# Lapis-Hong/wide_deep

Hardware: NVIDIA H100
Metric: CTR examples/sec (train step) (higher is better)
Workload: dtype bf16x3 (fp32 operands split into bf16 hi+lo, 3 tensor-core products, fp32 accumulate; 2^-16)

## Files before the change

wide_deep_b200/csrc/gemm.cuh:

```cuda
#pragma once
#include <cuda.h>
#include <cuda_bf16.h>

#include "common.cuh"

namespace wd {

__device__ __forceinline__ float act_fwd(int kind, float z) {
    switch (kind) {
        case WD_ACT_RELU: return fmaxf(z, 0.f);
        case WD_ACT_RELU6: return fminf(fmaxf(z, 0.f), 6.f);
        case WD_ACT_SIGMOID: return 1.f / (1.f + expf(-z));
        case WD_ACT_TANH: return tanhf(z);
        case WD_ACT_LEAKY_RELU: return z > 0.f ? z : 0.2f * z;
        case WD_ACT_ELU: return z > 0.f ? z : expm1f(z);
        case WD_ACT_SELU: return 1.0507009873554805f * (z > 0.f ? z : 1.6732632423543772f * expm1f(z));
        case WD_ACT_SOFTPLUS: return fmaxf(z, 0.f) + log1pf(expf(-fabsf(z)));
        case WD_ACT_SOFTSIGN: return z / (1.f + fabsf(z));
    }
    return z;
}
__device__ __forceinline__ float act_bwd(int kind, float a) {
    switch (kind) {
        case WD_ACT_RELU: return a > 0.f ? 1.f : 0.f;
        case WD_ACT_RELU6: return (a > 0.f && a < 6.f) ? 1.f : 0.f;
        case WD_ACT_SIGMOID: return a * (1.f - a);
        case WD_ACT_TANH: return 1.f - a * a;
        case WD_ACT_LEAKY_RELU: return a > 0.f ? 1.f : 0.2f;
        case WD_ACT_ELU: return a > 0.f ? 1.f : a + 1.f;
        case WD_ACT_SELU: return a > 0.f ? 1.0507009873554805f : a + 1.0507009873554805f * 1.6732632423543772f;
        case WD_ACT_SOFTPLUS: return 1.f - expf(-a);
        case WD_ACT_SOFTSIGN: { float t = 1.f - fabsf(a); return t * t; }
    }
    return 1.f;
}

struct GemmA {
    int n;
    const float* ptr[kMaxSegs];
    int ld[kMaxSegs];
    int k[kMaxSegs];
    const __nv_bfloat16* hi[kMaxSegs];
    const __nv_bfloat16* lo[kMaxSegs];
};
struct GemmB {
    const float* ptr; int ld;
    const float *tf32_hi, *tf32_lo;
    const __nv_bfloat16 *hi, *lo;
};
enum { EPI_FWD = 0, EPI_STORE = 1, EPI_WGRAD = 2 };
struct Epi {
    float* C; int ldc;
    int accumulate;
    float* A_out; float* H_out; int ldh;
    float* HT; int ldt;
    const float *bias, *gamma, *beta;
    int n_logical, act, bn;
    int m_valid;
    int64_t split_stride;
    __nv_bfloat16 *Hs_hi, *Hs_lo;
    uint64_t reserved[5];
};

int tc_gemm(WdModel* m, int mode, const GemmA& A, const GemmB& B, int M, int N, const Epi& ep, int splits, int ksplit_len);
int tc_gemm_bf16(WdModel* m, int mode, const GemmA& A, const GemmB& B, int M, int N, const Epi& ep, int splits, int ksplit_len);
int make_tensor_map(CUtensorMap* map, CUtensorMapDataType dtype, const void* ptr, int rows, int cols, int ld, int box_rows);

struct DropArgs { float rate; unsigned long long seed; const unsigned int* step; int layer_id; unsigned int row0; };
__device__ __forceinline__ unsigned long long splitmix64_dev(unsigned long long x) {
    x += 0x9E3779B97F4A7C15ULL;
    x = (x ^ (x >> 30)) * 0xBF58476D1CE4E5B9ULL;
    x = (x ^ (x >> 27)) * 0x94D049BB133111EBULL;
    return x ^ (x >> 31);
}
__device__ __forceinline__ unsigned long long drop_key(const DropArgs& d) {
    return splitmix64_dev(d.seed ^ ((unsigned long long)(*d.step) * 0x9E3779B97F4A7C15ULL) ^ ((unsigned long long)d.layer_id << 48));
}
__device__ __forceinline__ float drop_mult(unsigned long long key, unsigned int m, unsigned int n, float rate, float inv_keep) {
    const unsigned long long r = splitmix64_dev(key ^ ((unsigned long long)m * 65536ULL + n));
    const float u = (float)(unsigned int)(r >> 40) * (1.f / 16777216.f);
    return u >= rate ? inv_keep : 0.f;
}

__device__ __forceinline__ float bn_out(float a, const float* __restrict__ gamma, const float* __restrict__ beta, int n, int bn) {
    return bn ? fmaf(a, gamma[n] * 0.99950037468777f, beta[n]) : a;
}

__device__ __forceinline__ void split_bf16(float x, __nv_bfloat16& hi, __nv_bfloat16& lo) {
    hi = __float2bfloat16_rn(x);
    lo = __float2bfloat16_rn(x - __bfloat162float(hi));
}
__device__ __forceinline__ void split_pair(float x0, float x1, uint32_t& hi, uint32_t& lo) {
    const __nv_bfloat162 hp = __floats2bfloat162_rn(x0, x1);
    hi = *reinterpret_cast<const uint32_t*>(&hp);
    const __nv_bfloat162 lp = __floats2bfloat162_rn(x0 - __uint_as_float(hi << 16), x1 - __uint_as_float(hi & 0xFFFF0000u));
    lo = *reinterpret_cast<const uint32_t*>(&lp);
}
__device__ __forceinline__ void store_split4(__nv_bfloat16* hi, __nv_bfloat16* lo, float x0, float x1, float x2, float x3) {
    uint2 ph, pl;
    split_pair(x0, x1, ph.x, pl.x);
    split_pair(x2, x3, ph.y, pl.y);
    *reinterpret_cast<uint2*>(hi) = ph;
    *reinterpret_cast<uint2*>(lo) = pl;
}

}
```

wide_deep_b200/csrc/gemm_bf16.cu:

```cuda
#include <cuda.h>
#include <stdlib.h>

#include <algorithm>
#include <type_traits>

#include "common.cuh"
#include "gemm.cuh"
#include "wgmma_ptx.cuh"

namespace wd {

namespace {

constexpr int QBM = 128;
constexpr int QBN = 128;
constexpr int QNST = 3;
constexpr int QBK = 64;
constexpr int Q_THREADS = 384;

struct QMaps {
    CUtensorMap a_hi[kMaxSegs], a_lo[kMaxSegs];
    CUtensorMap b_hi, b_lo;
};
struct QSegs { int n; int k[kMaxSegs]; int koff[kMaxSegs]; };

__device__ unsigned long long g_probe[32 * 8];
__device__ __forceinline__ unsigned long long gtime() { unsigned long long t; asm volatile("mov.u64 %0, %globaltimer;" : "=l"(t)); return t; }
#define PROBE(i) do { if (probe >= 0 && blockIdx.x == 0 && (threadIdx.x & 127) == 0) g_probe[probe * 8 + (i)] = gtime(); } while (0)

template <int MODE>
__global__ void __launch_bounds__(Q_THREADS, 1) tc_gemm_bf16_kernel(const __grid_constant__ QMaps maps, const QSegs segs, int M, int N, int ktot,
                                                                   int ksplit_len, int nsplit, Epi ep, int probe) {
    extern __shared__ uint8_t smem_raw[];
    uint8_t* base = reinterpret_cast<uint8_t*>((reinterpret_cast<uintptr_t>(smem_raw) + 1023) & ~uintptr_t(1023));
    constexpr bool A_MN = MODE == EPI_WGRAD;
    constexpr bool B_MN = MODE == EPI_FWD || MODE == EPI_WGRAD;
    constexpr int A_BYTES = QBM * 128, B_BYTES = QBN * 128;
    constexpr int STAGE_BYTES = 2 * (A_BYTES + B_BYTES);
    auto a_hi = [&](int s) { return base + s * STAGE_BYTES; };
    auto a_lo = [&](int s) { return base + s * STAGE_BYTES + A_BYTES; };
    auto b_hi = [&](int s) { return base + s * STAGE_BYTES + 2 * A_BYTES; };
    auto b_lo = [&](int s) { return base + s * STAGE_BYTES + 2 * A_BYTES + B_BYTES; };
    uint64_t* bars = reinterpret_cast<uint64_t*>(base + QNST * STAGE_BYTES);
    uint64_t* full = bars; uint64_t* empty = bars + QNST;
    float* epi_vec = reinterpret_cast<float*>(base + QNST * STAGE_BYTES + 64);

    const int warp = threadIdx.x >> 5, lane = threadIdx.x & 31, wg = threadIdx.x >> 7;
    const int tiles_n = (N + QBN - 1) / QBN, tiles_m = (M + QBM - 1) / QBM;
    const int ntiles = tiles_n * tiles_m * nsplit;
    int nkb_all = 0;
    for (int s = 0; s < segs.n; ++s) nkb_all += (segs.k[s] + QBK - 1) / QBK;
    auto tile_range = [&](int tile, int& m0, int& n0, int& z, int& kbeg, int& nkb) {
        z = tile / (tiles_n * tiles_m);
        int r = tile % (tiles_n * tiles_m);
        m0 = (r / tiles_n) * QBM;
        n0 = (r % tiles_n) * QBN;
        kbeg = 0;
        nkb = nkb_all;
        if (MODE == EPI_WGRAD) {
            kbeg = z * ksplit_len;
            int kend = min(ktot, kbeg + ksplit_len);
            nkb = kend > kbeg ? (kend - kbeg + QBK - 1) / QBK : 0;
        }
    };

    if (threadIdx.x == 0) {
        for (int s = 0; s < QNST; ++s) { mbar_init(&full[s], 1); mbar_init(&empty[s], 8); }
        asm volatile("fence.mbarrier_init.release.cluster;" ::: "memory");
    }
    __syncthreads();

    if (wg == 0) {
        reg_dealloc<40>();
        PROBE(0);
        if (warp == 0 && lane == 0) {
            int g = 0;
            for (int tile = blockIdx.x; tile < ntiles; tile += gridDim.x) {
                int m0, n0, z, kbeg, nkb;
                tile_range(tile, m0, n0, z, kbeg, nkb);
                int seg = 0, kin = 0;
                for (int kb = 0; kb < nkb; ++kb, ++g) {
                    const int s = g % QNST, it = g / QNST;
                    if (it > 0) mbar_wait(&empty[s], (it - 1) & 1);
                    int ka, kbcoord;
                    if (MODE == EPI_WGRAD) { ka = kbeg + kb * QBK; kbcoord = ka; }
                    else {
                        if (kin >= segs.k[seg]) { ++seg; kin = 0; }
                        ka = kin; kbcoord = segs.koff[seg] + kin;
                        kin += QBK;
                    }
                    mbar_expect_tx(&full[s], 2 * (A_BYTES + B_BYTES));
                    if (!A_MN) {
                        tma_load_2d(a_hi(s), &maps.a_hi[seg], &full[s], ka, m0);
                        tma_load_2d(a_lo(s), &maps.a_lo[seg], &full[s], ka, m0);
                    } else {
#pragma unroll
                        for (int i = 0; i < QBM / 64; ++i) {
                            tma_load_2d(a_hi(s) + i * 8192, &maps.a_hi[seg], &full[s], m0 + 64 * i, ka);
                            tma_load_2d(a_lo(s) + i * 8192, &maps.a_lo[seg], &full[s], m0 + 64 * i, ka);
                        }
                    }
                    if (!B_MN) {
                        tma_load_2d(b_hi(s), &maps.b_hi, &full[s], kbcoord, n0);
                        tma_load_2d(b_lo(s), &maps.b_lo, &full[s], kbcoord, n0);
                    } else {
#pragma unroll
                        for (int i = 0; i < QBN / 64; ++i) {
                            tma_load_2d(b_hi(s) + i * 8192, &maps.b_hi, &full[s], n0 + 64 * i, kbcoord);
                            tma_load_2d(b_lo(s) + i * 8192, &maps.b_lo, &full[s], n0 + 64 * i, kbcoord);
                        }
                    }
                }
            }
        }
    } else {
        reg_alloc<232>();
        const int cw = wg - 1, cwarp = warp - 4;
        constexpr uint32_t a_step = A_MN ? 2048u : 32u, b_step = B_MN ? 2048u : 32u;
        constexpr int TA = A_MN ? 1 : 0, TB = B_MN ? 1 : 0;
        float d[QBN / 2];
        int g = 0, use = 0;
        for (int tile = blockIdx.x; tile < ntiles; tile += gridDim.x) {
            int m0, n0, z, kbeg, nkb;
            tile_range(tile, m0, n0, z, kbeg, nkb);
            if (nkb == 0) {
#pragma unroll
                for (int i = 0; i < QBN / 2; ++i) d[i] = 0.f;
            }
            const int ct = threadIdx.x - 128;
            float pre[2] = {0.f, 0.f};
            if (MODE == EPI_FWD) {
#pragma unroll
                for (int i = 0; i < 2; ++i) {
                    const int v = ct + 256 * i, c = n0 + (v & 127);
                    const bool in = c < ep.n_logical;
                    if (v < 128) pre[i] = in ? __ldg(ep.bias + c) : 0.f;
                    else if (v < 256) pre[i] = (in && ep.bn) ? __ldg(ep.gamma + c) * 0.99950037468777f : 1.f;
                    else if (v < 384) pre[i] = (in && ep.bn) ? __ldg(ep.beta + c) : 0.f;
                }
            }
            int prev = -1;
            for (int kb = 0; kb < nkb; ++kb, ++g) {
                const int s = g % QNST, it = g / QNST;
                mbar_wait(&full[s], it & 1);
                if (g == 0) PROBE(1);
                const uint32_t sa_hi = smem_u32(a_hi(s)) + cw * 8192, sa_lo = smem_u32(a_lo(s)) + cw * 8192;
                const uint32_t sb_hi = smem_u32(b_hi(s)), sb_lo = smem_u32(b_lo(s));
                wgmma_fence();
#pragma unroll
                for (int k = 0; k < QBK / 16; ++k) {
                    const uint64_t da_hi = A_MN ? make_desc_mn(sa_hi + k * a_step) : make_desc(sa_hi + k * a_step);
                    const uint64_t da_lo = A_MN ? make_desc_mn(sa_lo + k * a_step) : make_desc(sa_lo + k * a_step);
                    const uint64_t db_hi = B_MN ? make_desc_mn(sb_hi + k * b_step) : make_desc(sb_hi + k * b_step);
                    const uint64_t db_lo = B_MN ? make_desc_mn(sb_lo + k * b_step) : make_desc(sb_lo + k * b_step);
                    wgmma_bf16<TA, TB>(d, da_lo, db_hi, (kb > 0 || k > 0) ? 1u : 0u);
                    wgmma_bf16<TA, TB>(d, da_hi, db_lo, 1u);
                    wgmma_bf16<TA, TB>(d, da_hi, db_hi, 1u);
                }
                wgmma_commit();
                if (prev >= 0) {
                    wgmma_wait<1>();
                    if (lane == 0) mbar_arrive(&empty[prev]);
                }
                prev = s;
            }
            wgmma_wait<0>();
            if (prev >= 0 && lane == 0) mbar_arrive(&empty[prev]);
            if (cwarp == 0) PROBE(use == 0 ? 2 : 3);
            const float* ev = epi_vec + (use & 1) * 384;
            if (MODE == EPI_FWD) {
                epi_vec[(use & 1) * 384 + ct] = pre[0];
                if (ct < 128) epi_vec[(use & 1) * 384 + ct + 256] = pre[1];
                bar_sync(1, 256);
            }

            const int r0 = m0 + cw * 64 + (warp & 3) * 16 + (lane >> 2);
            const int cq = 2 * (lane & 3);
            auto epilogue = [&](auto relu) {
                constexpr bool RELU = decltype(relu)::value;
                uint32_t qh[2][2] = {}, ql[2][2] = {};
#pragma unroll
                for (int j = 0; j < QBN / 8; ++j) {
                    const int c = n0 + 8 * j + cq;
                    if (n0 + 8 * j < N) {
                        if (MODE == EPI_FWD) {
                            const bool in0 = c < ep.n_logical, in1 = c + 1 < ep.n_logical;
                            const int cl = 8 * j + cq;
                            const float b0 = ev[cl], b1 = ev[cl + 1], g0 = ev[128 + cl], g1 = ev[129 + cl], e0 = ev[256 + cl], e1 = ev[257 + cl];
#pragma unroll
                            for (int hh = 0; hh < 2; ++hh) {
                                const int r = r0 + 8 * hh;
                                if (r >= M) continue;
                                const bool rv = r < ep.m_valid;
                                float a0 = 0.f, a1 = 0.f, h0 = 0.f, h1 = 0.f;
                                if (rv && in0) { a0 = RELU ? fmaxf(d[4 * j + 2 * hh] + b0, 0.f) : act_fwd(ep.act, d[4 * j + 2 * hh] + b0); h0 = fmaf(a0, g0, e0); }
                                if (rv && in1) { a1 = RELU ? fmaxf(d[4 * j + 2 * hh + 1] + b1, 0.f) : act_fwd(ep.act, d[4 * j + 2 * hh + 1] + b1); h1 = fmaf(a1, g1, e1); }
                                const int64_t o = (int64_t)r * ep.ldh + c;
                                if (ep.A_out != ep.H_out) *reinterpret_cast<float2*>(ep.A_out + o) = make_float2(a0, a1);
                                if (ep.H_out) *reinterpret_cast<float2*>(ep.H_out + o) = make_float2(h0, h1);
                                split_pair(h0, h1, qh[j & 1][hh], ql[j & 1][hh]);
                            }
                            if (j & 1) {
                                const int q = lane & 3, src = (lane & ~3) + 2 * (q & 1);
                                const int64_t cp = n0 + 16 * (j >> 1) + 4 * q;
#pragma unroll
                                for (int hh = 0; hh < 2; ++hh) {
                                    uint2 vh, vl;
                                    const uint32_t h0a = __shfl_sync(0xffffffffu, qh[0][hh], src), h1a = __shfl_sync(0xffffffffu, qh[1][hh], src);
                                    const uint32_t h0b = __shfl_sync(0xffffffffu, qh[0][hh], src + 1), h1b = __shfl_sync(0xffffffffu, qh[1][hh], src + 1);
                                    const uint32_t l0a = __shfl_sync(0xffffffffu, ql[0][hh], src), l1a = __shfl_sync(0xffffffffu, ql[1][hh], src);
                                    const uint32_t l0b = __shfl_sync(0xffffffffu, ql[0][hh], src + 1), l1b = __shfl_sync(0xffffffffu, ql[1][hh], src + 1);
                                    vh.x = q < 2 ? h0a : h1a; vh.y = q < 2 ? h0b : h1b;
                                    vl.x = q < 2 ? l0a : l1a; vl.y = q < 2 ? l0b : l1b;
                                    const int r = r0 + 8 * hh;
                                    if (r >= M) continue;
                                    const int64_t o = (int64_t)r * ep.ldh + cp;
                                    *reinterpret_cast<uint2*>(ep.Hs_hi + o) = vh;
                                    *reinterpret_cast<uint2*>(ep.Hs_lo + o) = vl;
                                }
                            }
                        } else {
                            float* Cb = ep.C + (MODE == EPI_WGRAD ? (int64_t)z * ep.split_stride : 0);
#pragma unroll
                            for (int hh = 0; hh < 2; ++hh) {
                                const int r = r0 + 8 * hh;
                                if (r >= M) continue;
                                float2* pc = reinterpret_cast<float2*>(Cb + (int64_t)r * ep.ldc + c);
                                float2 o = make_float2(d[4 * j + 2 * hh], d[4 * j + 2 * hh + 1]);
                                if (MODE == EPI_STORE && ep.accumulate) { const float2 p = *pc; o.x += p.x; o.y += p.y; }
                                *pc = o;
                            }
                        }
                    }
                }
            };
            if (MODE == EPI_FWD && ep.act == WD_ACT_RELU) epilogue(std::true_type{});
            else epilogue(std::false_type{});
            if (cwarp == 0) PROBE(use == 0 ? 4 : 5);
            ++use;
        }
    }
}

int g_probe_slot = 0;

template <int MODE>
int launch_q(WdModel* m, const QMaps& maps, const QSegs& segs, int M, int N, int ktot, int splits, int ksplit_len, const Epi& ep) {
    constexpr int smem = QNST * 2 * (QBM * 128 + QBN * 128) + 1024 + 64 + 2 * 384 * 4;
    static bool configured = false;
    static int num_sms = 0;
    if (!configured) {
        WD_CUDA(cudaFuncSetAttribute(tc_gemm_bf16_kernel<MODE>, cudaFuncAttributeMaxDynamicSharedMemorySize, smem));
        WD_CUDA(cudaDeviceGetAttribute(&num_sms, cudaDevAttrMultiProcessorCount, m->device));
        configured = true;
    }
    const int nsplit = MODE == EPI_WGRAD ? splits : 1;
    const int ntiles = ((N + QBN - 1) / QBN) * ((M + QBM - 1) / QBM) * nsplit;
    static const bool probe_on = getenv("WD_GEMM_PROBE") != nullptr;
    const int probe = probe_on ? (g_probe_slot++ & 31) : -1;
    tc_gemm_bf16_kernel<MODE><<<ntiles < num_sms ? ntiles : num_sms, Q_THREADS, smem, m->stream>>>(maps, segs, M, N, ktot, ksplit_len, nsplit, ep, probe);
    m->launches++;
    WD_CUDA(cudaGetLastError());
    return WD_OK;
}

}

extern "C" int wd_debug_gemm_probe(unsigned long long* out) {
    cudaDeviceSynchronize();
    cudaError_t e = cudaMemcpyFromSymbol(out, g_probe, sizeof(unsigned long long) * 32 * 8);
    g_probe_slot = 0;
    return e == cudaSuccess ? 0 : -1;
}

int tc_gemm_bf16(WdModel* m, int mode, const GemmA& A, const GemmB& B, int M, int N, const Epi& ep, int splits, int ksplit_len) {
    constexpr CUtensorMapDataType BF16 = CU_TENSOR_MAP_DATA_TYPE_BFLOAT16;
    if (N % 32 != 0 || A.n > kMaxSegs || !B.hi || !B.lo) { set_error("bf16 GEMM engine: unsupported operands"); return WD_EUNSUPPORTED; }
    QMaps maps;
    QSegs segs{};
    segs.n = A.n;
    int rc, ktot = 0;
    const bool a_mn = mode == EPI_WGRAD, b_mn = mode == EPI_FWD || mode == EPI_WGRAD;
    for (int s = 0; s < A.n; ++s) {
        if (!A.hi[s] || !A.lo[s]) { set_error("bf16 GEMM engine: operand without hi/lo copies"); return WD_EINVAL; }
        if (!a_mn) {
            if ((rc = make_tensor_map(&maps.a_hi[s], BF16, A.hi[s], M, A.k[s], A.ld[s], QBM))) return rc;
            if ((rc = make_tensor_map(&maps.a_lo[s], BF16, A.lo[s], M, A.k[s], A.ld[s], QBM))) return rc;
        } else {
            if ((rc = make_tensor_map(&maps.a_hi[s], BF16, A.hi[s], A.k[s], M, A.ld[s], 64))) return rc;
            if ((rc = make_tensor_map(&maps.a_lo[s], BF16, A.lo[s], A.k[s], M, A.ld[s], 64))) return rc;
        }
        segs.k[s] = A.k[s]; segs.koff[s] = ktot;
        ktot += A.k[s];
    }
    for (int s = A.n; s < kMaxSegs; ++s) { maps.a_hi[s] = maps.a_hi[0]; maps.a_lo[s] = maps.a_lo[0]; }
    if (!b_mn) {
        if ((rc = make_tensor_map(&maps.b_hi, BF16, B.hi, N, ktot, B.ld, QBN))) return rc;
        if ((rc = make_tensor_map(&maps.b_lo, BF16, B.lo, N, ktot, B.ld, QBN))) return rc;
    } else {
        if ((rc = make_tensor_map(&maps.b_hi, BF16, B.hi, ktot, N, B.ld, 64))) return rc;
        if ((rc = make_tensor_map(&maps.b_lo, BF16, B.lo, ktot, N, B.ld, 64))) return rc;
    }
    if (mode == EPI_WGRAD) ksplit_len = (ksplit_len + QBK - 1) / QBK * QBK;
    if (mode == EPI_FWD && (!ep.Hs_hi || !ep.Hs_lo)) { set_error("bf16 GEMM engine: epilogue without hi/lo outputs"); return WD_EINVAL; }
    if (mode == EPI_FWD) return launch_q<EPI_FWD>(m, maps, segs, M, N, ktot, splits, ksplit_len, ep);
    if (mode == EPI_STORE) return launch_q<EPI_STORE>(m, maps, segs, M, N, ktot, splits, ksplit_len, ep);
    return launch_q<EPI_WGRAD>(m, maps, segs, M, N, ktot, splits, ksplit_len, ep);
}

}
```

wide_deep_b200/csrc/mlp.cu:

```cuda
#include "common.cuh"
#include "gemm.cuh"

namespace wd {

constexpr int BM = 128, BN = 128, BK = 16, GT = 256;

template <int MODE>
__global__ void __launch_bounds__(GT) gemm_tn_ffma(GemmA A, const float* __restrict__ Bm, int ldb, int M, int N, int ksplit_len, Epi ep) {
    __shared__ __align__(16) float As[2][BK][BM + 4];
    __shared__ __align__(16) float Bs[2][BK][BN + 4];
    const int tid = threadIdx.x, tx = tid & 15, ty = tid >> 4;
    const int m0 = blockIdx.y * BM, n0 = blockIdx.x * BN;
    float acc[8][8];
#pragma unroll
    for (int i = 0; i < 8; ++i)
#pragma unroll
        for (int j = 0; j < 8; ++j) acc[i][j] = 0.f;

    int ktot = 0;
    for (int s = 0; s < A.n; ++s) ktot += A.k[s];
    int kbeg = 0, kend = ktot;
    if (MODE == EPI_WGRAD) {
        kbeg = blockIdx.z * ksplit_len;
        kend = min(ktot, kbeg + ksplit_len);
// ... 72 lines not shown
                            a = act_fwd(ep.act, acc[ih * 4 + i][jh * 4 + j] + ep.bias[gn]);
                            h = bn_out(a, ep.gamma, ep.beta, gn, ep.bn);
                        }
                        a4[j] = a;
                        hv[i][j] = h;
                    }
                    if (gm < M) {
                        if (ep.A_out != ep.H_out)
                            *reinterpret_cast<float4*>(ep.A_out + (int64_t)gm * ep.ldh + nb) = make_float4(a4[0], a4[1], a4[2], a4[3]);
                        *reinterpret_cast<float4*>(ep.H_out + (int64_t)gm * ep.ldh + nb) = make_float4(hv[i][0], hv[i][1], hv[i][2], hv[i][3]);
                    }
                }
                if (ep.HT) {
#pragma unroll
                    for (int j = 0; j < 4; ++j)
                        *reinterpret_cast<float4*>(ep.HT + (int64_t)(nb + j) * ep.ldt + mb) = make_float4(hv[0][j], hv[1][j], hv[2][j], hv[3][j]);
                }
            } else {
                float* Cb = ep.C + (MODE == EPI_WGRAD ? (int64_t)blockIdx.z * ep.split_stride : 0);
#pragma unroll
                for (int i = 0; i < 4; ++i) {
                    const int gm = mb + i;
                    if (gm >= M) continue;
                    float4 v = make_float4(acc[ih * 4 + i][jh * 4 + 0], acc[ih * 4 + i][jh * 4 + 1], acc[ih * 4 + i][jh * 4 + 2], acc[ih * 4 + i][jh * 4 + 3]);
                    float4* dst = reinterpret_cast<float4*>(Cb + (int64_t)gm * ep.ldc + nb);
                    if (MODE == EPI_STORE && ep.accumulate) {
                        float4 o = *dst;
                        v.x += o.x; v.y += o.y; v.z += o.z; v.w += o.w;
                    }
                    *dst = v;
                }
            }
        }
    }
}

static void launch_gemm(WdModel* m, int mode, const GemmA& A, const GemmB& B, int M, int N, const Epi& ep, int splits, int ksplit_len) {
    dim3 grid((N + BN - 1) / BN, (M + BM - 1) / BM, mode == EPI_WGRAD ? splits : 1);
    if (mode == EPI_FWD) gemm_tn_ffma<EPI_FWD><<<grid, GT, 0, m->stream>>>(A, B.ptr, B.ld, M, N, 0, ep);
    else if (mode == EPI_STORE) gemm_tn_ffma<EPI_STORE><<<grid, GT, 0, m->stream>>>(A, B.ptr, B.ld, M, N, 0, ep);
    else gemm_tn_ffma<EPI_WGRAD><<<grid, GT, 0, m->stream>>>(A, B.ptr, B.ld, M, N, ksplit_len, ep);
    m->launches++;
}

static int run_gemm(WdModel* m, int mode, const GemmA& A, const GemmB& B, int M, int N, const Epi& ep, int splits = 1, int ksplit_len = 0) {
    static const char* kNamesL[3][4] = {{"gemm_fwd_l0", "gemm_fwd_l1", "gemm_fwd_l2", "gemm_fwd_l3+"},
                                        {"gemm_dgrad_l0", "gemm_dgrad_l1", "gemm_dgrad_l2", "gemm_dgrad_l3+"},
                                        {"gemm_wgrad_l0", "gemm_wgrad_l1", "gemm_wgrad_l2", "gemm_wgrad_l3+"}};
    const char* kNames[3] = {kNamesL[0][m->cur_layer < 3 ? m->cur_layer : 3], kNamesL[1][m->cur_layer < 3 ? m->cur_layer : 3],
                             kNamesL[2][m->cur_layer < 3 ? m->cur_layer : 3]};
    mark(m, "mlp_other");
    if (m->operands == kBf16Operands) {
        int rc = tc_gemm_bf16(m, mode, A, B, M, N, ep, splits, ksplit_len);
        mark(m, kNames[mode]);
        return rc;
    }
    if (m->gemm_engine == WD_GEMM_TC3X || m->gemm_engine == WD_GEMM_TC1X) {
        int rc = tc_gemm(m, mode, A, B, M, N, ep, splits, ksplit_len);
        if (rc != WD_EUNSUPPORTED) { mark(m, kNames[mode]); return rc; }
        m->gemm_fallbacks++;
        static bool warned = false;
        if (!warned) { fprintf(stderr, "libwd_b200: wgmma engine does not cover a GEMM (M=%d N=%d segs=%d): running it on the FFMA kernel\n", M, N, A.n); warned = true; }
    }
    launch_gemm(m, mode, A, B, M, N, ep, splits, ksplit_len);
    mark(m, kNames[mode]);
    return WD_OK;
}

__global__ void transpose_kernel(const float* __restrict__ in, int ld_in, int M, int Mpad, int N, float* __restrict__ out, int ld_out) {
    __shared__ float t[32][33];
    int m0 = blockIdx.y * 32, n0 = blockIdx.x * 32;
    for (int i = threadIdx.y; i < 32; i += 8) {
        int mm = m0 + i, nn = n0 + threadIdx.x;
        t[i][threadIdx.x] = (mm < M && nn < N) ? in[(int64_t)mm * ld_in + nn] : 0.f;
    }
    __syncthreads();
    for (int i = threadIdx.y; i < 32; i += 8) {
        int nn = n0 + i, mm = m0 + threadIdx.x;
        if (nn < N && mm < Mpad) out[(int64_t)nn * ld_out + mm] = t[threadIdx.x][i];
    }
}

__global__ void x0_split_kernel(const float* __restrict__ in, int64_t n4, __nv_bfloat16* __restrict__ hi, __nv_bfloat16* __restrict__ lo) {
    for (int64_t i = (int64_t)blockIdx.x * blockDim.x + threadIdx.x; i < n4; i += (int64_t)gridDim.x * blockDim.x) {
        const float4 x = reinterpret_cast<const float4*>(in)[i];
        store_split4(hi + 4 * i, lo + 4 * i, x.x, x.y, x.z, x.w);
    }
}

__global__ void __launch_bounds__(256) dropout_fwd_kernel(int B, int N, int n_logical, const float* __restrict__ A, int ld,
                                                         const float* __restrict__ gamma, const float* __restrict__ beta, int bn,
                                                         float* __restrict__ H, __nv_bfloat16* __restrict__ q_hi, __nv_bfloat16* __restrict__ q_lo,
                                                         float* __restrict__ HT, int ldt, DropArgs dr) {
    const unsigned long long key = drop_key(dr);
    const float inv_keep = 1.f / (1.f - dr.rate);
    const int64_t total = (int64_t)B * N;
    for (int64_t t = (int64_t)blockIdx.x * blockDim.x + threadIdx.x; t < total; t += (int64_t)gridDim.x * blockDim.x) {
        const int mrow = (int)(t / N), n = (int)(t % N);
        float h = 0.f;
        if (n < n_logical) {
            const float a = A[(int64_t)mrow * ld + n] * drop_mult(key, dr.row0 + (unsigned)mrow, (unsigned)n, dr.rate, inv_keep);
            h = bn_out(a, gamma, beta, n, bn);
        }
        if (H) H[(int64_t)mrow * ld + n] = h;
        if (q_hi) {
            __nv_bfloat16 hh, hl;
            split_bf16(h, hh, hl);
// ... 152 lines not shown
            if (mm < B && n < N) dZ[(int64_t)mm * ld + n] = dz;
            tile[ty * 4 + i][tx] = dz;
        }
        __syncthreads();
#pragma unroll
        for (int i = 0; i < 4; ++i) {
            int nn = blockIdx.x * 32 + ty * 4 + i;
            if (nn < N) dZT[(int64_t)nn * ldt + mbase + tx] = tile[tx][ty * 4 + i];
        }
        __syncthreads();
    }
    red[0][ty][tx] = sb; red[1][ty][tx] = sg; red[2][ty][tx] = sbe;
    __syncthreads();
    if (ty == 0 && n < N) {
        float a = 0.f, b = 0.f, c = 0.f;
        for (int i = 0; i < 8; ++i) { a += red[0][i][tx]; b += red[1][i][tx]; c += red[2][i][tx]; }
        p_bias[(int64_t)rt * pstride + n] = a;
        if (bn) { p_gamma[(int64_t)rt * pstride + n] = b; p_beta[(int64_t)rt * pstride + n] = c; }
    }
}

__global__ void __launch_bounds__(256) act_bn_bwd_q_kernel(int B, int N, int n_logical, const float* __restrict__ dH, const float* __restrict__ Aact,
                                                          int ld, const float* __restrict__ gamma, int act, int bn,
                                                          float* __restrict__ p_bias, float* __restrict__ p_gamma, float* __restrict__ p_beta,
                                                          int64_t pstride, __nv_bfloat16* __restrict__ q_hi, __nv_bfloat16* __restrict__ q_lo, DropArgs dr) {
    __shared__ float red[3][16][64];
    const unsigned long long dkey = dr.rate > 0.f ? drop_key(dr) : 0ull;
    const float inv_keep = dr.rate > 0.f ? 1.f / (1.f - dr.rate) : 1.f;
    const int cx = threadIdx.x & 15, ry = threadIdx.x >> 4;
    const int n0 = blockIdx.x * 64 + cx * 4, rt = blockIdx.y, b0 = rt * 128;
    const float inv = 0.99950037468777f;
    float gsc[4], sb[4] = {0.f, 0.f, 0.f, 0.f}, sg[4] = {0.f, 0.f, 0.f, 0.f}, sbe[4] = {0.f, 0.f, 0.f, 0.f};
#pragma unroll
    for (int j = 0; j < 4; ++j) gsc[j] = (bn && n0 + j < n_logical) ? gamma[n0 + j] * inv : 1.f;
    if (n0 < N) {
        float4 dhv[8], av[8];
#pragma unroll
        for (int u = 0; u < 8; ++u) {
            const int mr = min(b0 + u * 16 + ry, B - 1);
            dhv[u] = *reinterpret_cast<const float4*>(dH + (int64_t)mr * ld + n0);
            av[u] = *reinterpret_cast<const float4*>(Aact + (int64_t)mr * ld + n0);
        }
#pragma unroll
        for (int u = 0; u < 8; ++u) {
            const int mm = b0 + u * 16 + ry;
            if (mm >= B) continue;
            const float dh[4] = {dhv[u].x, dhv[u].y, dhv[u].z, dhv[u].w}, a[4] = {av[u].x, av[u].y, av[u].z, av[u].w};
            float dz[4];
#pragma unroll
            for (int j = 0; j < 4; ++j) {
                dz[j] = 0.f;
                if (n0 + j < n_logical) {
                    const float dm = dr.rate > 0.f ? drop_mult(dkey, dr.row0 + (unsigned)mm, (unsigned)(n0 + j), dr.rate, inv_keep) : 1.f;
                    dz[j] = dh[j] * gsc[j] * dm * act_bwd(act, a[j]);
                    sb[j] += dz[j]; sg[j] += dh[j] * (a[j] * dm) * inv; sbe[j] += dh[j];
                }
            }
            store_split4(q_hi + (int64_t)mm * ld + n0, q_lo + (int64_t)mm * ld + n0, dz[0], dz[1], dz[2], dz[3]);
        }
    }
#pragma unroll
    for (int j = 0; j < 4; ++j) { red[0][ry][cx * 4 + j] = sb[j]; red[1][ry][cx * 4 + j] = sg[j]; red[2][ry][cx * 4 + j] = sbe[j]; }
    __syncthreads();
    if (threadIdx.x < 192) {
        const int which = threadIdx.x >> 6, c = threadIdx.x & 63, n = blockIdx.x * 64 + c;
        if (n < N && (which == 0 || bn)) {
            float x = 0.f;
#pragma unroll
            for (int i = 0; i < 16; ++i) x += red[which][i][c];
            (which == 0 ? p_bias : which == 1 ? p_gamma : p_beta)[(int64_t)rt * pstride + n] = x;
        }
    }
}

__global__ void __launch_bounds__(256) logits_act_bwd_q_kernel(int B, int N, int n_logical, const float* __restrict__ H, int ldh,
                                                              const float* __restrict__ Aact, int ld, const float* __restrict__ dlogit,
                                                              const float* __restrict__ kw, const float* __restrict__ gamma, int act, int bn,
                                                              float* __restrict__ p_kw, int64_t kw_stride, float* __restrict__ p_lbias, int64_t lbias_stride,
                                                              float* __restrict__ p_wbias, int64_t wbias_stride,
                                                              float* __restrict__ p_bias, float* __restrict__ p_gamma, float* __restrict__ p_beta, int64_t pstride,
                                                              __nv_bfloat16* __restrict__ q_hi, __nv_bfloat16* __restrict__ q_lo) {
    __shared__ float red[4][16][64];
    __shared__ float dl[128];
    const int cx = threadIdx.x & 15, ry = threadIdx.x >> 4;
    const int n0 = blockIdx.x * 64 + cx * 4, rt = blockIdx.y, b0 = rt * 128;
    const float inv = 0.99950037468777f;
    if (threadIdx.x < 128) dl[threadIdx.x] = (b0 + threadIdx.x < B) ? dlogit[b0 + threadIdx.x] : 0.f;
    float gsc[4], w[4], sk[4] = {0.f, 0.f, 0.f, 0.f}, sb[4] = {0.f, 0.f, 0.f, 0.f}, sg[4] = {0.f, 0.f, 0.f, 0.f}, sbe[4] = {0.f, 0.f, 0.f, 0.f};
#pragma unroll
    for (int j = 0; j < 4; ++j) {
        gsc[j] = (bn && n0 + j < n_logical) ? gamma[n0 + j] * inv : 1.f;
        w[j] = n0 + j < N ? kw[n0 + j] : 0.f;
    }
    __syncthreads();
    if (n0 < N) {
        float4 hv[8], av[8];
#pragma unroll
        for (int u = 0; u < 8; ++u) {
            const int mr = min(b0 + u * 16 + ry, B - 1);
            hv[u] = *reinterpret_cast<const float4*>(H + (int64_t)mr * ldh + n0);
            av[u] = *reinterpret_cast<const float4*>(Aact + (int64_t)mr * ld + n0);
        }
#pragma unroll
        for (int u = 0; u < 8; ++u) {
            const int mm = b0 + u * 16 + ry;
            if (mm >= B) continue;
            const float g = dl[u * 16 + ry];
            const float h[4] = {hv[u].x, hv[u].y, hv[u].z, hv[u].w}, a[4] = {av[u].x, av[u].y, av[u].z, av[u].w};
// ... 295 lines not shown
                dropout_fwd_kernel<<<grid_for((int64_t)B * L.N_phys, 256), 256, 0, m->stream>>>(B, L.N_phys, L.N, L.A, L.N_phys, ep.gamma, ep.beta, m->batch_norm,
                    L.H, L.Hs[0], L.Hs[1], ep.HT, m->ldt, dr);
                m->launches++;
            }
        }
    }
    WD_CUDA(cudaGetLastError());
    return WD_OK;
}

int loss_forward(WdModel* m, bool need_grad) {
    const int B = m->dbatch.B;
    const int ntow = m->use_deep ? (int)m->towers.size() : 0;
    HeadIn in{};
    in.n = ntow;
    for (int t = 0; t < ntow; ++t) {
        Tower& tw = m->towers[t];
        Layer& LL = tw.layers[tw.n_hidden];
        in.S[t].n = LL.n_in_segs;
        for (int s = 0; s < LL.n_in_segs; ++s) {
            in.S[t].ptr[s] = src_ptr(m, tw, LL.segs[s].src);
            in.S[t].ld[s] = src_ld(m, tw, LL.segs[s].src);
            in.S[t].k[s] = LL.segs[s].width_phys;
            in.S[t].koff[s] = LL.segs[s].k_off;
        }
        in.kernel[t] = m->d_P + m->dense[LL.t_kernel].off;
        in.bias[t] = m->d_P + m->dense[LL.t_bias].off;
        in.tower_logit[t] = tw.logit;
    }
    const int blocks = grid_for((int64_t)B * 8, 256, 512);
    logits_head_kernel<<<blocks, 256, 0, m->stream>>>(in, B, m->use_wide ? m->d_wide_logit : nullptr, m->dbatch.label,
                                                     m->dbatch.weight, m->d_logits, need_grad ? m->d_dlogit : nullptr, m->d_loss_part,
                                                     m->d_head_counter, m->d_loss);
    m->launches++;
    WD_CUDA(cudaGetLastError());
    return WD_OK;
}

int mlp_backward(WdModel* m) {
    const int B = m->dbatch.B;
    if (!m->use_deep) return WD_OK;
    const int rts = (B + 127) / 128;
    const int Bk = (B + 15) / 16 * 16;
    bool dx0_written = false;
    const bool need_dx0 = !m->tables.empty();
    const bool bf16_ops = m->operands == kBf16Operands;
    for (auto& tw : m->towers) {
        std::vector<char> written(tw.n_hidden, 0);
        std::vector<int> readers(tw.n_hidden, 0);
        std::vector<char> fused(tw.n_hidden, 0);
        for (int l = 0; l <= tw.n_hidden; ++l)
            for (int s = 0; s < tw.layers[l].n_in_segs; ++s)
                if (tw.layers[l].segs[s].src >= 0) readers[tw.layers[l].segs[s].src] += (l == tw.n_hidden ? 2 : 1);
        auto grad_dst = [&](int src, float** p, int* ld, int* acc) {
            if (src < 0) { *p = m->d_dX0; *ld = m->d0_phys; *acc = dx0_written ? 1 : 0; dx0_written = true; }
            else { *p = tw.layers[src].dH; *ld = tw.layers[src].N_phys; *acc = written[src] ? 1 : 0; written[src] = 1; }
        };
        Layer& LL = tw.layers[tw.n_hidden];
        const DenseTensor& tk = m->dense[LL.t_kernel];
        const DenseTensor& tb = m->dense[LL.t_bias];
        for (int s = 0; s < LL.n_in_segs; ++s) {
            const Seg& sg = LL.segs[s];
            const float* src = src_ptr(m, tw, sg.src);
            int ld = src_ld(m, tw, sg.src);
            dim3 g((sg.width_phys + 63) / 64, rts);
            float* dst = nullptr; int dld = 0, acc = 0;
            if (!(sg.src < 0 && !need_dx0)) grad_dst(sg.src, &dst, &dld, &acc);
            const bool wb = m->use_wide && s == 0 && &tw == &m->towers.front();
            if (bf16_ops && LL.n_in_segs == 1 && sg.src >= 0 && readers[sg.src] == 2 && m->dropout_rate <= 0.f &&
                sg.width_phys == tw.layers[sg.src].N_phys) {
                Layer& S = tw.layers[sg.src];
                logits_act_bwd_q_kernel<<<dim3((S.N_phys + 63) / 64, rts), 256, 0, m->stream>>>(B, S.N_phys, S.N, src, ld, S.A, S.N_phys, m->d_dlogit,
                    m->d_P + tk.off + sg.k_off, S.t_gamma >= 0 ? m->d_P + m->dense[S.t_gamma].off : nullptr, m->activation, m->batch_norm,
                    m->d_gpart + tk.gpart_off + sg.k_off, tk.gstride, m->d_gpart + tb.gpart_off, tb.gstride,
                    wb ? m->d_gpart + m->dense[0].gpart_off : nullptr, wb ? m->dense[0].gstride : 0,
                    m->d_gpart + m->dense[S.t_bias].gpart_off, S.t_gamma >= 0 ? m->d_gpart + m->dense[S.t_gamma].gpart_off : nullptr,
                    S.t_beta >= 0 ? m->d_gpart + m->dense[S.t_beta].gpart_off : nullptr, m->dense[S.t_bias].gstride, S.dZs[0], S.dZs[1]);
                m->launches++;
                fused[sg.src] = 1;
                continue;
            }
            logits_bwd_kernel<<<g, 256, 0, m->stream>>>(B, sg.width_phys, src, ld, m->d_dlogit, m->d_P + tk.off + sg.k_off,
                                                       m->d_gpart + tk.gpart_off + sg.k_off, tk.gstride,
                                                       s == 0 ? m->d_gpart + tb.gpart_off : nullptr, tb.gstride,
                                                       wb ? m->d_gpart + m->dense[0].gpart_off : nullptr, wb ? m->dense[0].gstride : 0, dst, dld, acc);
            m->launches++;
        }
        for (int l = tw.n_hidden - 1; l >= 0; --l) {
            Layer& L = tw.layers[l];
            m->cur_layer = l;
            float* pb = m->d_gpart + m->dense[L.t_bias].gpart_off;
            float* pg = L.t_gamma >= 0 ? m->d_gpart + m->dense[L.t_gamma].gpart_off : nullptr;
            float* pbe = L.t_beta >= 0 ? m->d_gpart + m->dense[L.t_beta].gpart_off : nullptr;
            if (!written[l] && !fused[l]) {
                WD_CUDA(cudaMemsetAsync(L.dH, 0, (size_t)m->max_batch_pad * L.N_phys * sizeof(float), m->stream));
            }
            dim3 g((L.N_phys + 31) / 32, rts);
            const DropArgs dr{m->dropout_rate, m->dropout_seed, m->d_step, (int)(&tw - &m->towers[0]) * 64 + l, drop_row0(m)};
            if (fused[l]) {
            } else if (bf16_ops)
                act_bn_bwd_q_kernel<<<dim3((L.N_phys + 63) / 64, rts), 256, 0, m->stream>>>(B, L.N_phys, L.N, L.dH, L.A, L.N_phys,
                    L.t_gamma >= 0 ? m->d_P + m->dense[L.t_gamma].off : nullptr, m->activation, m->batch_norm, pb, pg, pbe,
                    m->dense[L.t_bias].gstride, L.dZs[0], L.dZs[1], dr);
            else
            act_bn_bwd_kernel<<<g, 256, 0, m->stream>>>(B, L.N_phys, L.N, L.dH, L.A, L.N_phys,
                                                       L.t_gamma >= 0 ? m->d_P + m->dense[L.t_gamma].off : nullptr, m->activation,
                                                       m->batch_norm, L.dZ, L.dZT, m->ldt, pb, pg, pbe, m->dense[L.t_bias].gstride, dr);
            if (!fused[l]) m->launches++;
            for (int s = 0; s < L.n_in_segs; ++s) {
                const Seg& sg = L.segs[s];
                if (sg.src < 0 && !need_dx0) continue;
                float* dst; int dld, acc;
                grad_dst(sg.src, &dst, &dld, &acc);
                GemmA A{}; GemmB W{};
                dgrad_operands(m, L, sg, A, W);
                Epi ep{};
                ep.C = dst; ep.ldc = dld; ep.accumulate = acc;
                int rc = run_gemm(m, EPI_STORE, A, W, B, sg.width_phys, ep);
                if (rc) return rc;
            }
            if (l == 0 && &tw == &m->towers.back() && need_dx0 && m->ev_dx0 && m->record_dx0) {
                WD_CUDA(cudaEventRecord(m->ev_dx0, m->stream));
                m->dx0_recorded = true;
            }
        }
        for (int l = tw.n_hidden - 1; l >= 0; --l) {
            Layer& L = tw.layers[l];
            m->cur_layer = l;
            const DenseTensor& tkn = m->dense[L.t_kernel];
            if (l == 0 && m->record_wgrad_rest && m->towers.size() == 1 && L.n_in_segs == 1) {
                WD_CUDA(cudaEventRecord(m->ev_wgrad_rest, m->stream));
                m->dense_split_tensor = L.t_kernel;
            }
            for (int s = 0; s < L.n_in_segs; ++s) {
                const Seg& sg = L.segs[s];
                GemmA A{}; GemmB W{};
                wgrad_operands(m, tw, L, sg, A, W);
                Epi ep{};
                ep.C = m->d_gpart + tkn.gpart_off + (int64_t)sg.k_off * L.N_phys; ep.ldc = L.N_phys; ep.split_stride = tkn.gstride;
                const int ks = ((Bk + L.wgrad_splits - 1) / L.wgrad_splits + 31) / 32 * 32;
                int rc = run_gemm(m, EPI_WGRAD, A, W, sg.width_phys, L.N_phys, ep, L.wgrad_splits, ks);
                if (rc) return rc;
            }
        }
    }
    WD_CUDA(cudaGetLastError());
    return WD_OK;
}

__global__ void crelu_fold_kernel(float* __restrict__ gp, int parts, int64_t gstride, int rows, int cols, int u) {
    const int64_t total = (int64_t)parts * rows * u;
    for (int64_t i = (int64_t)blockIdx.x * blockDim.x + threadIdx.x; i < total; i += (int64_t)gridDim.x * blockDim.x) {
        const int n = (int)(i % u);
        const int64_t pr = i / u;
        float* q = gp + (pr / rows) * gstride + (pr % rows) * cols + n;
        q[0] -= q[u];
        q[u] = 0.f;
    }
}
__global__ void crelu_mirror_kernel(float* __restrict__ P, float* __restrict__ S1, float* __restrict__ S2, int rows, int cols, int u) {
    const int64_t total = (int64_t)rows * u;
    for (int64_t i = (int64_t)blockIdx.x * blockDim.x + threadIdx.x; i < total; i += (int64_t)gridDim.x * blockDim.x) {
        const int64_t e = (i / u) * cols + i % u;
        P[e + u] = -P[e];
        S1[e + u] = S1[e];
        S2[e + u] = S2[e];
    }
}
static int crelu_fold(WdModel* m) {
    const int rts = (m->dbatch.B + 127) / 128;
    for (const DenseTensor& t : m->dense) {
// ... 80 lines not shown
```

Baseline: 10.47 million.

## Fuse activation/BN backward into dgrad GEMM epilogue for single-reader layers

Adds an EPI_DACT epilogue mode to the bf16x3 GEMM. In this mode the dgrad output dH is consumed in registers: the activation derivative and BN scale are applied, dZ is split into bf16 hi/lo, and per-tile bias/gamma/beta partial sums are reduced through shared memory. This removes the separate act_bn_bwd_q kernel launch and the dH write and re-read for layers whose gradient comes from a single reader with no dropout. In exchange the epilogue uses more shared memory and adds extra barriers, and apre holds many preloaded activation values in registers.

```diff
diff --git a/wide_deep_b200/csrc/gemm.cuh b/wide_deep_b200/csrc/gemm.cuh
--- a/wide_deep_b200/csrc/gemm.cuh
+++ b/wide_deep_b200/csrc/gemm.cuh
@@ -48,7 +48,7 @@
     const float *tf32_hi, *tf32_lo;
     const __nv_bfloat16 *hi, *lo;
 };
-enum { EPI_FWD = 0, EPI_STORE = 1, EPI_WGRAD = 2 };
+enum { EPI_FWD = 0, EPI_STORE = 1, EPI_WGRAD = 2, EPI_DACT = 3 };
 struct Epi {
     float* C; int ldc;
     int accumulate;
@@ -59,7 +59,9 @@
     int m_valid;
     int64_t split_stride;
     __nv_bfloat16 *Hs_hi, *Hs_lo;
-    uint64_t reserved[5];
+    const float* act_in;
+    float *p_bias, *p_gamma, *p_beta;
+    int64_t pstride;
 };
 
 int tc_gemm(WdModel* m, int mode, const GemmA& A, const GemmB& B, int M, int N, const Epi& ep, int splits, int ksplit_len);
@@ -86,6 +88,11 @@
     return bn ? fmaf(a, gamma[n] * 0.99950037468777f, beta[n]) : a;
 }
 
+__device__ __forceinline__ void act_bn_bwd_elem(float dh, float a, float gsc, float dm, int act, float& dz, float& t) {
+    dz = dh * gsc * dm * act_bwd(act, a);
+    t = dh * (a * dm);
+}
+
 __device__ __forceinline__ void split_bf16(float x, __nv_bfloat16& hi, __nv_bfloat16& lo) {
     hi = __float2bfloat16_rn(x);
     lo = __float2bfloat16_rn(x - __bfloat162float(hi));
diff --git a/wide_deep_b200/csrc/gemm_bf16.cu b/wide_deep_b200/csrc/gemm_bf16.cu
--- a/wide_deep_b200/csrc/gemm_bf16.cu
+++ b/wide_deep_b200/csrc/gemm_bf16.cu
@@ -17,6 +17,8 @@
 constexpr int QNST = 3;
 constexpr int QBK = 64;
 constexpr int Q_THREADS = 384;
+constexpr int Q_SMEM = QNST * 2 * (QBM * 128 + QBN * 128) + 1024 + 64 + 2 * 384 * 4;
+constexpr int Q_DACT_SMEM = (3 * 8 * 256 + 3 * 256) * 4;
 
 struct QMaps {
     CUtensorMap a_hi[kMaxSegs], a_lo[kMaxSegs];
@@ -44,6 +46,8 @@
     uint64_t* bars = reinterpret_cast<uint64_t*>(base + QNST * STAGE_BYTES);
     uint64_t* full = bars; uint64_t* empty = bars + QNST;
     float* epi_vec = reinterpret_cast<float*>(base + QNST * STAGE_BYTES + 64);
+    float* dact_terms = epi_vec + 2 * 384;
+    float* dact_usum = dact_terms + 3 * 8 * 256;
 
     const int warp = threadIdx.x >> 5, lane = threadIdx.x & 31, wg = threadIdx.x >> 7;
     const int tiles_n = (N + QBN - 1) / QBN, tiles_m = (M + QBM - 1) / QBM;
@@ -129,6 +133,19 @@
             }
             const int ct = threadIdx.x - 128;
             float pre[2] = {0.f, 0.f};
+            float2 apre[MODE == EPI_DACT ? QBN / 8 : 1][2];
+            if (MODE == EPI_DACT) {
+                const int r0 = m0 + cw * 64 + (warp & 3) * 16 + (lane >> 2), cq = 2 * (lane & 3);
+                if (ct < 128) pre[0] = (ep.bn && n0 + ct < ep.n_logical) ? __ldg(ep.gamma + n0 + ct) * 0.99950037468777f : 1.f;
+#pragma unroll
+                for (int j = 0; j < QBN / 8; ++j)
+#pragma unroll
+                    for (int hh = 0; hh < 2; ++hh) {
+                        const int r = r0 + 8 * hh;
+                        apre[j][hh] = (r < ep.m_valid && n0 + 8 * j < N)
+                                          ? __ldg(reinterpret_cast<const float2*>(ep.act_in + (int64_t)r * ep.ldc + n0 + 8 * j + cq)) : make_float2(0.f, 0.f);
+                    }
+            }
             if (MODE == EPI_FWD) {
 #pragma unroll
                 for (int i = 0; i < 2; ++i) {
@@ -171,6 +188,10 @@
             if (MODE == EPI_FWD) {
                 epi_vec[(use & 1) * 384 + ct] = pre[0];
                 if (ct < 128) epi_vec[(use & 1) * 384 + ct + 256] = pre[1];
+                bar_sync(1, 256);
+            }
+            if (MODE == EPI_DACT) {
+                if (ct < 128) epi_vec[(use & 1) * 384 + ct] = pre[0];
                 bar_sync(1, 256);
             }
 
@@ -200,6 +221,26 @@
                                 if (ep.H_out) *reinterpret_cast<float2*>(ep.H_out + o) = make_float2(h0, h1);
                                 split_pair(h0, h1, qh[j & 1][hh], ql[j & 1][hh]);
                             }
+                        } else if (MODE == EPI_DACT) {
+                            const bool in0 = c < ep.n_logical, in1 = c + 1 < ep.n_logical;
+                            const float g0 = ev[8 * j + cq], g1 = ev[8 * j + cq + 1];
+                            const int u = 4 * cw + (warp & 3);
+#pragma unroll
+                            for (int hh = 0; hh < 2; ++hh) {
+                                const int r = r0 + 8 * hh;
+                                const bool rv = r < ep.m_valid;
+                                const float dh0 = d[4 * j + 2 * hh], dh1 = d[4 * j + 2 * hh + 1];
+                                float z0 = 0.f, z1 = 0.f, t0 = 0.f, t1 = 0.f, e0 = 0.f, e1 = 0.f;
+                                if (rv && in0) { act_bn_bwd_elem(dh0, apre[j][hh].x, g0, 1.f, RELU ? WD_ACT_RELU : ep.act, z0, t0); e0 = dh0; }
+                                if (rv && in1) { act_bn_bwd_elem(dh1, apre[j][hh].y, g1, 1.f, RELU ? WD_ACT_RELU : ep.act, z1, t1); e1 = dh1; }
+                                split_pair(z0, z1, qh[j & 1][hh], ql[j & 1][hh]);
+                                const int o = u * 256 + ((j & 1) * 16 + (lane >> 2) + 8 * hh) * 8 + cq;
+                                *reinterpret_cast<float2*>(dact_terms + o) = make_float2(z0, z1);
+                                *reinterpret_cast<float2*>(dact_terms + 2048 + o) = make_float2(t0, t1);
+                                *reinterpret_cast<float2*>(dact_terms + 4096 + o) = make_float2(e0, e1);
+                            }
+                        }
+                        if (MODE == EPI_FWD || MODE == EPI_DACT) {
                             if (j & 1) {
                                 const int q = lane & 3, src = (lane & ~3) + 2 * (q & 1);
                                 const int64_t cp = n0 + 16 * (j >> 1) + 4 * q;
@@ -219,6 +260,28 @@
                                     *reinterpret_cast<uint2*>(ep.Hs_lo + o) = vl;
                                 }
                             }
+                            if (MODE == EPI_DACT && (j & 1)) {
+                                bar_sync(1, 256);
+                                {
+                                    float sb = 0.f, sg = 0.f, sbe = 0.f;
+#pragma unroll
+                                    for (int u = 0; u < 8; ++u) {
+                                        sb += dact_terms[u * 256 + ct];
+                                        sg = fmaf(dact_terms[2048 + u * 256 + ct], 0.99950037468777f, sg);
+                                        sbe += dact_terms[4096 + u * 256 + ct];
+                                    }
+                                    dact_usum[ct] = sb; dact_usum[256 + ct] = sg; dact_usum[512 + ct] = sbe;
+                                }
+                                bar_sync(1, 256);
+                                const int which = ct >> 4, n = n0 + 16 * (j >> 1) + (ct & 15);
+                                if (ct < 48 && (which == 0 || ep.bn)) {
+                                    const float* us = dact_usum + which * 256 + (ct & 8) * 16 + (ct & 7);
+                                    float x = 0.f;
+#pragma unroll
+                                    for (int ry = 0; ry < 16; ++ry) x += us[ry * 8];
+                                    (which == 0 ? ep.p_bias : which == 1 ? ep.p_gamma : ep.p_beta)[(int64_t)(m0 / QBM) * ep.pstride + n] = x;
+                                }
+                            }
                         } else {
                             float* Cb = ep.C + (MODE == EPI_WGRAD ? (int64_t)z * ep.split_stride : 0);
 #pragma unroll
@@ -234,7 +297,7 @@
                     }
                 }
             };
-            if (MODE == EPI_FWD && ep.act == WD_ACT_RELU) epilogue(std::true_type{});
+            if ((MODE == EPI_FWD || MODE == EPI_DACT) && ep.act == WD_ACT_RELU) epilogue(std::true_type{});
             else epilogue(std::false_type{});
             if (cwarp == 0) PROBE(use == 0 ? 4 : 5);
             ++use;
@@ -246,7 +309,7 @@
 
 template <int MODE>
 int launch_q(WdModel* m, const QMaps& maps, const QSegs& segs, int M, int N, int ktot, int splits, int ksplit_len, const Epi& ep) {
-    constexpr int smem = QNST * 2 * (QBM * 128 + QBN * 128) + 1024 + 64 + 2 * 384 * 4;
+    constexpr int smem = Q_SMEM + (MODE == EPI_DACT ? Q_DACT_SMEM : 0);
     static bool configured = false;
     static int num_sms = 0;
     if (!configured) {
@@ -303,7 +366,12 @@
     }
     if (mode == EPI_WGRAD) ksplit_len = (ksplit_len + QBK - 1) / QBK * QBK;
     if (mode == EPI_FWD && (!ep.Hs_hi || !ep.Hs_lo)) { set_error("bf16 GEMM engine: epilogue without hi/lo outputs"); return WD_EINVAL; }
+    if (mode == EPI_DACT && (!ep.Hs_hi || !ep.Hs_lo || !ep.act_in || !ep.p_bias || (ep.bn && (!ep.p_gamma || !ep.p_beta || !ep.gamma)))) {
+        set_error("bf16 GEMM engine: activation-backward epilogue without its inputs or outputs");
+        return WD_EINVAL;
+    }
     if (mode == EPI_FWD) return launch_q<EPI_FWD>(m, maps, segs, M, N, ktot, splits, ksplit_len, ep);
+    if (mode == EPI_DACT) return launch_q<EPI_DACT>(m, maps, segs, M, N, ktot, splits, ksplit_len, ep);
     if (mode == EPI_STORE) return launch_q<EPI_STORE>(m, maps, segs, M, N, ktot, splits, ksplit_len, ep);
     return launch_q<EPI_WGRAD>(m, maps, segs, M, N, ktot, splits, ksplit_len, ep);
 }
diff --git a/wide_deep_b200/csrc/mlp.cu b/wide_deep_b200/csrc/mlp.cu
--- a/wide_deep_b200/csrc/mlp.cu
+++ b/wide_deep_b200/csrc/mlp.cu
@@ -148,7 +148,7 @@
     mark(m, "mlp_other");
     if (m->operands == kBf16Operands) {
         int rc = tc_gemm_bf16(m, mode, A, B, M, N, ep, splits, ksplit_len);
-        mark(m, kNames[mode]);
+        mark(m, kNames[mode == EPI_DACT ? EPI_STORE : mode]);
         return rc;
     }
     if (m->gemm_engine == WD_GEMM_TC3X || m->gemm_engine == WD_GEMM_TC1X) {
@@ -407,8 +407,9 @@
                 dz[j] = 0.f;
                 if (n0 + j < n_logical) {
                     const float dm = dr.rate > 0.f ? drop_mult(dkey, dr.row0 + (unsigned)mm, (unsigned)(n0 + j), dr.rate, inv_keep) : 1.f;
-                    dz[j] = dh[j] * gsc[j] * dm * act_bwd(act, a[j]);
-                    sb[j] += dz[j]; sg[j] += dh[j] * (a[j] * dm) * inv; sbe[j] += dh[j];
+                    float t;
+                    act_bn_bwd_elem(dh[j], a[j], gsc[j], dm, act, dz[j], t);
+                    sb[j] += dz[j]; sg[j] = fmaf(t, inv, sg[j]); sbe[j] += dh[j];
                 }
             }
             store_split4(q_hi + (int64_t)mm * ld + n0, q_lo + (int64_t)mm * ld + n0, dz[0], dz[1], dz[2], dz[3]);
@@ -810,6 +811,13 @@
         for (int l = 0; l <= tw.n_hidden; ++l)
             for (int s = 0; s < tw.layers[l].n_in_segs; ++s)
                 if (tw.layers[l].segs[s].src >= 0) readers[tw.layers[l].segs[s].src] += (l == tw.n_hidden ? 2 : 1);
+        std::vector<char> dact(tw.n_hidden, 0);
+        if (bf16_ops && m->dropout_rate <= 0.f && !m->crelu)
+            for (int l = 0; l < tw.n_hidden; ++l)
+                for (int s = 0; s < tw.layers[l].n_in_segs; ++s) {
+                    const Seg& sg = tw.layers[l].segs[s];
+                    if (sg.src >= 0 && readers[sg.src] == 1 && sg.width_phys == tw.layers[sg.src].N_phys) dact[sg.src] = 1;
+                }
         auto grad_dst = [&](int src, float** p, int* ld, int* acc) {
             if (src < 0) { *p = m->d_dX0; *ld = m->d0_phys; *acc = dx0_written ? 1 : 0; dx0_written = true; }
             else { *p = tw.layers[src].dH; *ld = tw.layers[src].N_phys; *acc = written[src] ? 1 : 0; written[src] = 1; }
@@ -855,7 +863,7 @@
             }
             dim3 g((L.N_phys + 31) / 32, rts);
             const DropArgs dr{m->dropout_rate, m->dropout_seed, m->d_step, (int)(&tw - &m->towers[0]) * 64 + l, drop_row0(m)};
-            if (fused[l]) {
+            if (fused[l] || dact[l]) {
             } else if (bf16_ops)
                 act_bn_bwd_q_kernel<<<dim3((L.N_phys + 63) / 64, rts), 256, 0, m->stream>>>(B, L.N_phys, L.N, L.dH, L.A, L.N_phys,
                     L.t_gamma >= 0 ? m->d_P + m->dense[L.t_gamma].off : nullptr, m->activation, m->batch_norm, pb, pg, pbe,
@@ -864,7 +872,7 @@
             act_bn_bwd_kernel<<<g, 256, 0, m->stream>>>(B, L.N_phys, L.N, L.dH, L.A, L.N_phys,
                                                        L.t_gamma >= 0 ? m->d_P + m->dense[L.t_gamma].off : nullptr, m->activation,
                                                        m->batch_norm, L.dZ, L.dZT, m->ldt, pb, pg, pbe, m->dense[L.t_bias].gstride, dr);
-            if (!fused[l]) m->launches++;
+            if (!fused[l] && !dact[l]) m->launches++;
             for (int s = 0; s < L.n_in_segs; ++s) {
                 const Seg& sg = L.segs[s];
                 if (sg.src < 0 && !need_dx0) continue;
@@ -874,7 +882,18 @@
                 dgrad_operands(m, L, sg, A, W);
                 Epi ep{};
                 ep.C = dst; ep.ldc = dld; ep.accumulate = acc;
-                int rc = run_gemm(m, EPI_STORE, A, W, B, sg.width_phys, ep);
+                if (sg.src >= 0 && dact[sg.src]) {
+                    const Layer& S = tw.layers[sg.src];
+                    ep.C = nullptr;
+                    ep.act_in = S.A; ep.gamma = S.t_gamma >= 0 ? m->d_P + m->dense[S.t_gamma].off : nullptr;
+                    ep.act = m->activation; ep.bn = m->batch_norm; ep.n_logical = S.N; ep.m_valid = B;
+                    ep.Hs_hi = S.dZs[0]; ep.Hs_lo = S.dZs[1]; ep.ldh = S.N_phys;
+                    ep.p_bias = m->d_gpart + m->dense[S.t_bias].gpart_off;
+                    ep.p_gamma = S.t_gamma >= 0 ? m->d_gpart + m->dense[S.t_gamma].gpart_off : nullptr;
+                    ep.p_beta = S.t_beta >= 0 ? m->d_gpart + m->dense[S.t_beta].gpart_off : nullptr;
+                    ep.pstride = m->dense[S.t_bias].gstride;
+                }
+                int rc = run_gemm(m, sg.src >= 0 && dact[sg.src] ? EPI_DACT : EPI_STORE, A, W, B, sg.width_phys, ep);
                 if (rc) return rc;
             }
             if (l == 0 && &tw == &m->towers.back() && need_dx0 && m->ev_dx0 && m->record_dx0) {
```

Result: faster. 10.64 million, median of 6 (+1.6%).
